# mitrefireline/simfire

Hardware: AMD Instinct MI355X
Metric: cell-updates/sec (grid x envs x steps) (higher is better)
Workload: dtype u8 status + u8 sprite masks + f64 burn_amounts

## Files before the change

profiles/isa_waits.py:

```python
#!/usr/bin/env python3
import argparse
import os
import re
import subprocess
import sys
import tempfile

ROOT = os.path.dirname(os.path.dirname(os.path.abspath(__file__)))
MEM = re.compile(r"^\s*(global_|flat_|scratch_|buffer_|ds_|s_load_|s_buffer_load_)")
LABEL = re.compile(r"^(\.LBB\d+_\d+):")
DPP_START = "wave_shr:1"
ROW_LOAD = "global_load_dwordx4"


def compile_asm(unit, out):
    sys.path.insert(0, ROOT)
    from simfire_amd import build as B
    hipcc = os.environ.get("HIPCC", "/opt/rocm/bin/hipcc")
    flags = [f for f in B.FLAGS if f != "-shared"] + ["-S", "--cuda-device-only"]
    subprocess.run([hipcc] + flags + ["-o", out, os.path.join(B.CSRC, unit)], check=True, stderr=subprocess.DEVNULL)
    return out


def mangled(args):
# ... 65 lines not shown
    skip, every = vm_waits_on_skip_path(body, load, dpp), vm_waits_between(body, load, dpp)
    p("# vmcnt waits between them: %d on the path that takes every s_cbranch_execz, %d on any path" % (len(skip), len(every)))
    p("# index | wait | memory instructions issued since the wait before (x count)")
    pending = []
    for i in range(first, last):
        op = instr(body[i])
        if i == load - 3:
            p("%6d | -- prefetch: the next batch's four rows are requested here" % i)
        if i == dpp:
            p("%6d | -- the batch's work starts (first %s)" % (i, DPP_START))
        if MEM.match(op):
            pending.append(op.split()[0])
        elif op.startswith("s_waitcnt"):
            seen = []
            for m_ in pending:
                if seen and seen[-1][0] == m_:
                    seen[-1][1] += 1
                else:
                    seen.append([m_, 1])
            p("%6d | %-32s | %s" % (i, op, " ".join(n if c == 1 else "%s x%d" % (n, c) for n, c in seen) or "-"))
            pending = []


def main():
    ap = argparse.ArgumentParser(description=__doc__.split("\n")[0])
    ap.add_argument("--unit", default="simfire_hip_run2.hip")
    ap.add_argument("--kernel", default="1,0,1,0,2", help="template arguments of k_run: MAXD,ATT,DIAG,MIT,TEAM")
    ap.add_argument("--asm", default=None)
    a = ap.parse_args()
    if a.asm:
        text = open(a.asm).read()
    else:
        with tempfile.TemporaryDirectory() as d:
            text = open(compile_asm(a.unit, os.path.join(d, "unit.s"))).read()
    report(kernel_lines(text, a.kernel), a.kernel)


if __name__ == "__main__":
    main()
```

simfire_amd/csrc/sf_run_kernels.h:

```cpp
#pragma once

#include "sf_common.h"
#include "sf_step_kernels.h"

namespace {

constexpr int kMarkDw = 32;
constexpr int kStripDw = 19;
#ifdef SF_NO_PERM_ELIG
#define ELIG(x) elig01(x)
#else
#define ELIG(x) elig01_perm(x)
#endif
constexpr int kRunCtl = 24;
constexpr int kRunMaxD = 4;

typedef uint32_t __attribute__((aligned(1))) u32_unaligned;
typedef uint32_t u32x4 __attribute__((ext_vector_type(4)));

__host__ __device__ inline size_t win_lds_bytes(int n_waves)
{
    const int WR = n_waves * 4;
    return (size_t)WR * 64 * 8 + 8 * 8 * 4 + 128 * 4 + 64 * 4 + (size_t)(WR + 2) * 18 * 4 + (size_t)WR * 16 + (size_t)2 * WR * 64 * 2 + (size_t)2 * WR * 64 +
           (size_t)WR * 64 + (size_t)WR * 8 + 256 * 4;
// ... 260 lines not shown
    const void *ka = (const void *)__builtin_amdgcn_kernarg_segment_ptr();
    uint32_t d0 = 0, d1 = 0, d2 = 0, d3 = 0, d4 = 0, d5 = 0, d6 = 0, d7 = 0, d8 = 0, d9 = 0, d10 = 0, d11 = 0, d12 = 0, d13 = 0, d14 = 0, d15 = 0;
    static_assert(BYTES <= 16 * 64, "more lines than this touches");
    d0 = kernarg_line<0>(ka);
    if (BYTES > 1 * 64) d1 = kernarg_line<1 * 64>(ka);
    if (BYTES > 2 * 64) d2 = kernarg_line<2 * 64>(ka);
    if (BYTES > 3 * 64) d3 = kernarg_line<3 * 64>(ka);
    if (BYTES > 4 * 64) d4 = kernarg_line<4 * 64>(ka);
    if (BYTES > 5 * 64) d5 = kernarg_line<5 * 64>(ka);
    if (BYTES > 6 * 64) d6 = kernarg_line<6 * 64>(ka);
    if (BYTES > 7 * 64) d7 = kernarg_line<7 * 64>(ka);
    if (BYTES > 8 * 64) d8 = kernarg_line<8 * 64>(ka);
    if (BYTES > 9 * 64) d9 = kernarg_line<9 * 64>(ka);
    if (BYTES > 10 * 64) d10 = kernarg_line<10 * 64>(ka);
    if (BYTES > 11 * 64) d11 = kernarg_line<11 * 64>(ka);
    if (BYTES > 12 * 64) d12 = kernarg_line<12 * 64>(ka);
    if (BYTES > 13 * 64) d13 = kernarg_line<13 * 64>(ka);
    if (BYTES > 14 * 64) d14 = kernarg_line<14 * 64>(ka);
    if (BYTES > 15 * 64) d15 = kernarg_line<15 * 64>(ka);
    asm volatile("s_waitcnt lgkmcnt(0)" : "+s"(d0), "+s"(d1), "+s"(d2), "+s"(d3), "+s"(d4), "+s"(d5), "+s"(d6), "+s"(d7), "+s"(d8), "+s"(d9), "+s"(d10), "+s"(d11), "+s"(d12),
                 "+s"(d13), "+s"(d14), "+s"(d15));
}

template <int MAXD, int ATT, int DIAG, int MIT, int TEAM = 0>
__global__ __launch_bounds__(1024) void k_run(StepArgs a_by_value, const int n_steps_launch, int vcap, int bsz)
{
    kernarg_touch<(int)sizeof(StepArgs) + 12>();
#ifdef SF_ARGS_BY_VALUE
    constexpr bool kArgsByValue = true;
#else
    constexpr bool kArgsByValue = TEAM == 2 || MIT == -2 || (MIT == 0 && TEAM == 0) || (TEAM == 1 && MAXD == 2);
#endif
    const StepArgs &a = kArgsByValue ? a_by_value : *(const StepArgs *)__builtin_amdgcn_kernarg_segment_ptr();
    extern __shared__ uint4 s_dyn[];
    const Geo &g = a.g;
    const int tid = threadIdx.x, wave = tid >> 6, lane = tid & 63, n_waves = blockDim.x >> 6, nthr = blockDim.x;
    int e_ = 0, tm_ = 0, tn_ = 1;
    bool no_work = false;
    if (TEAM) {
        const uint32_t tt = a.team_tab[blockIdx.x];
        if (tt == kTeamUnused) { if (TEAM != 2) return; no_work = true; }
        else { e_ = (int)(tt & 0xFFFFu); tm_ = (int)((tt >> 16) & 0xFFu); tn_ = (int)(tt >> 24); }
    } else if (a.todo_cnt) {
        const uint32_t n_left = *a.todo_cnt;
        if (blockIdx.x >= n_left) return;
        e_ = (int)a.todo_list[blockIdx.x];
    } else e_ = a.order ? (int)a.order[blockIdx.x] : (int)blockIdx.x;
    int j_s0 = -1;
    for (bool first_pass = true;; first_pass = false) {
    if (TEAM == 2 && (!first_pass || no_work)) {
        if (a.team_recut >= n_steps_launch) return;
        uint32_t *sc = reinterpret_cast<uint32_t *>(s_dyn);
        JoinArgs ja;
        ja.xj = a.xj; ja.xcut = a.xcut; ja.xerr = a.xerr; ja.E = g.E; ja.team_recut = a.team_recut; ja.join_floor = a.join_floor; ja.join_ovh = a.join_ovh;
        ja.team_timeout = a.team_timeout; ja.join_local = a.join_local; ja.t_cap = kTeamMax < g.TY ? kTeamMax : g.TY;
        const uint4 t = find_team(ja, sc);
// ... 169 lines not shown
        }
        __syncthreads();
        R0 = (int)tcnt[0]; R1 = (int)tcnt[1];
        const bool fits = __builtin_amdgcn_readfirstlane((int)tcnt[2]) != 0;
        R0 = __builtin_amdgcn_readfirstlane(R0); R1 = __builtin_amdgcn_readfirstlane(R1);
        if (R1 > g.H) R1 = g.H;
        __syncthreads();
        return fits;
    };
    {
        bool fits = true;
        if (TEAM && (tn > 1 || a.team_rcap) && general) fits = cut_bands(tn > 1 && a.team_recut > 0 && a.team_recut < n_steps ? a.team_recut : n_steps - s_begin);
        if (TEAM && a.todo_out && tm == 0 && tid == 0) a.todo_out[e] = fits ? 0 : n_steps - s_begin;
        if (TEAM && !fits) {
            if (!a.todo_out && tid == 0) *reinterpret_cast<volatile uint32_t *>(a.xerr) = 1u;
            if (s_begin > 0 && tm == 0 && tid == 0) a.commit[e] = st;
            return;
        }
    }
    bool has_up = TEAM && tm > 0, has_dn = TEAM && tm + 1 < tn;
    if (TEAM == 2 && tm == 0 && j_s0 < 0 && tid == 0)
        __hip_atomic_store(a.xj + 2 * g.E + 2 + e, (uint32_t)__builtin_amdgcn_s_getreg((20 << 0) | (0 << 6) | (31 << 11)) & 15u, __ATOMIC_RELAXED, __HIP_MEMORY_SCOPE_AGENT);
    auto team_release = [&]() {
        if (TEAM == 2 && a.join_local == 1) asm volatile("s_waitcnt vmcnt(0)" ::: "memory");
        else __builtin_amdgcn_fence(__ATOMIC_RELEASE, "agent");
    };
    auto team_acquire = [&]() { __builtin_amdgcn_fence(__ATOMIC_ACQUIRE, "agent"); };
    bool one_l2 = false;
    bool gave_up = false;
    auto line_up = [&](const uint32_t tag, const bool report) {
        typedef unsigned long long u64;
        int lane = threadIdx.x & 63;
        asm volatile("" : "+v"(lane));
        const uint32_t xcc = (uint32_t)__builtin_amdgcn_s_getreg((20 << 0) | (0 << 6) | (31 << 11)) & 15u;
        if (lane == 0) __hip_atomic_store(a.xg + ((size_t)e * kTeamMax + tm) * 3 + 2, ((u64)tag << 32) | (u64)xcc, __ATOMIC_RELAXED, __HIP_MEMORY_SCOPE_AGENT);
        u64 x = ((u64)tag << 32) | xcc;
        const unsigned long long t0 = __builtin_amdgcn_s_memrealtime();
        for (;;) {
            if (lane < tn) x = __hip_atomic_load(a.xg + ((size_t)e * kTeamMax + lane) * 3 + 2, __ATOMIC_RELAXED, __HIP_MEMORY_SCOPE_AGENT);
            if (__all((uint32_t)(x >> 32) >= tag)) break;
            __builtin_amdgcn_s_sleep(2);
            if (gave_up || __builtin_amdgcn_s_memrealtime() - t0 > a.team_timeout) {
                if (report) {
                    if (lane == 0) *reinterpret_cast<volatile uint32_t *>(a.xerr) = 1u;
                    gave_up = true;
                }
                break;
            }
        }
        one_l2 = __all((uint32_t)(x >> 32) >= tag && ((uint32_t)x & 15u) == xcc) && !a.team_far;
    };
    unsigned long long *vb = vb0, *vf = nullptr, *vl = nullptr, *ve = nullptr;
    auto load_band = [&]() {
        int tid = threadIdx.x;
        asm volatile("" : "+v"(tid));
        const int yoff = TEAM && a.team_rcap ? R0 - 1 : 0;
        vb = vb0 - (long long)yoff * VW;
        vf = fine ? vb + (size_t)lds_rows * VW : nullptr; vl = fine ? vb + (size_t)2 * lds_rows * VW : nullptr;
        ve = fine ? vb + (size_t)3 * lds_rows * VW : nullptr;
        const int y_lo = TEAM && a.team_rcap ? (R0 > 0 ? R0 - 1 : 0) : 0, y_hi = TEAM && a.team_rcap ? (R1 < g.H ? R1 + 1 : g.H) : g.H;
        for (int i = y_lo * VW + tid; i < y_hi * VW; i += nthr) {
            vb[i] = vb_glob[i];
            if (fine) {
                vf[i] = vb_glob[(long long)g.E * g.vb_env + i];
                vl[i] = vb_glob[2ll * g.E * g.vb_env + i];
                ve[i] = ~0ull;
            }
        }
        if (TEAM && tn > 1) {
            for (int i = tid; i < 2 * g.PV; i += nthr) {
                const int side = i >= g.PV, v = side ? i - g.PV : i, yh = side ? R1 : R0 - 1;
                uint4 r = make_uint4(0, 0, 0, 0);
                if (side ? has_dn : has_up)
                    r = *reinterpret_cast<const uint4 *>(a.cells + (long long)e * g.cells_env + bl_vec(g, yh, v) + (yh & 1) * 16);
                halo[i] = r;
            }
        }
    };
    if (general) load_band();
    PhaseClock pc;
#ifdef SF_PHASES
    uint32_t *ph_acc = ctl + kRunCtl + wave * 16;
    if (lane < 16) ph_acc[lane] = 0;
    pc.start(ph_acc);
#else
    pc.start();
#endif
    __syncthreads();
    if (TEAM == 1 && tn > 1) {
// ... 37 lines not shown
            __syncthreads();
            load_band();
            __syncthreads();
        }
    }
    if (TEAM && tn > 1) {
        if (wave == 0) line_up(TEAM == 2 && j_s0 >= 0 ? 2u + (uint32_t)(j_s0 / a.team_recut) : 1u, TEAM == 2 && j_s0 >= 0);
        if (TEAM == 2) __syncthreads();
    }

    RunEnv ev;
    ev.cells = a.cells + (long long)e * g.cells_env;
    ev.burn = a.burn + (long long)e * g.plane_env;
    ev.settled = a.settled ? a.settled + (long long)e * g.plane_env : nullptr;
    ev.rt = a.rt + (long long)e * g.rt_env;
    ev.vb = vb; ev.vf = vf; ev.vl = vl;
    ev.tdirty = a.tdirty + (long long)e * g.TY * g.TX;
    ev.tot = reinterpret_cast<int32_t *>(ctl + 10);
    int rpt = ((TEAM ? R1 - R0 : g.H) + nthr - 1) / nthr;
    int row0 = TEAM ? R0 : 0;
    auto store_band = [&]() {
        int tid = threadIdx.x;
        asm volatile("" : "+v"(tid));
        for (int i = R0 * VW + tid; i < R1 * VW; i += nthr) {
            vb_glob[i] = vb[i];
            vb_glob[(long long)g.E * g.vb_env + i] = vf[i];
            vb_glob[2ll * g.E * g.vb_env + i] = vl[i];
        }
    };
    const unsigned long long last_word_mask = (g.PV & 63) ? ((1ull << (g.PV & 63)) - 1ull) : ~0ull;

    const bool mit_one_wave = mit && a.mit_k <= 64;
    const int mit_wave = n_waves - 1;
    constexpr bool loop = MIT == -2;
    auto load_pt = [&](int s) {
        if (wave == mit_wave && lane < a.mit_k) {
            const int32_t *p = mit + (((long long)s * g.E + e) * a.mit_k + lane) * 3;
            px = p[0]; py = p[1]; pty = p[2];
        }
    };
    if (mit_one_wave && n_steps > 0 && !loop && !kWinMit) load_pt(0);
    uint32_t lseq = 0;
    if (loop) {
        if (tid == 0) ctl[18] = __hip_atomic_load(a.loop_done + e, __ATOMIC_RELAXED, __HIP_MEMORY_SCOPE_AGENT);
        __syncthreads();
        lseq = (uint32_t)__builtin_amdgcn_readfirstlane((int)ctl[18]);
        n_steps = 0x7FFFFFFF;
        counts_env(g, e, a.status, a.cells, a.tdirty, a.thist, st.running, st.steps, st.elapsed, a.res_block, a.res_elapsed, nullptr,
                   reinterpret_cast<int32_t (*)[6]>(vlist + vcap));
        if (tid == 0)
            for (int q = 0; q < 6; ++q) ev.tot[q] = a.res_block[e * 8 + 2 + q];
        if (e == 0 && a.mit_k > 0 && lseq > 0) {
            const int n16 = g.E * a.mit_k;
            const u32x4 *src = reinterpret_cast<const u32x4 *>(a.loop_pts_host) + (size_t)(lseq & 1u) * n16;
            u32x4 *cpy = reinterpret_cast<u32x4 *>(a.loop_pts) + (size_t)(lseq & 1u) * n16;
            for (int i = tid; i < n16; i += nthr) {
                u32x4 v;
                asm volatile("global_load_dwordx4 %0, %1, off sc0 sc1\n\ts_waitcnt vmcnt(0)" : "=&v"(v) : "v"(src + i) : "memory");
                if (v.w == lseq) asm volatile("global_store_dwordx4 %0, %1, off sc0 sc1" :: "v"(cpy + i), "v"(v) : "memory");
            }
        }
        __syncthreads();
    }
    unsigned long long join_clk = __builtin_readcyclecounter();
    unsigned long long x_clocks = 0;
    uint32_t x_steps = 0;
    for (int s = s_begin; s < n_steps && (st.running || mit); ++s) {
        const int k = s % 3, kn = (s + 1) % 3;
#ifdef SF_PHASES
        pc.tl = (e == g_timeline_env && s == g_timeline_step) ? g_timeline + wave * 64 : nullptr;
#endif
        auto loop_finish = [&]() {
            __syncthreads();
            if (tid == 0) {
                const int32_t *tot = ev.tot;
                int32_t *row = a.res_block + e * 8;
                row[0] = st.running == 1; row[1] = st.steps;
                for (int q = 0; q < 6; ++q) row[2 + q] = tot[q];
                a.res_elapsed[e] = st.elapsed;
            }
            ++lseq;
            if (wave == 0) {
                uint32_t *stage = strips;
                if (lane == 0) {
                    const int32_t *row = a.res_block + e * 8;
                    const unsigned long long el = (unsigned long long)__double_as_longlong(st.elapsed);
                    stage[0] = (uint32_t)row[0]; stage[1] = (uint32_t)row[1]; stage[2] = (uint32_t)row[2];
                    stage[4] = (uint32_t)row[3]; stage[5] = (uint32_t)row[4]; stage[6] = (uint32_t)row[5];
                    stage[8] = (uint32_t)row[6]; stage[9] = (uint32_t)row[7]; stage[10] = (uint32_t)el;
// ... 203 lines not shown
        }
        pc.mark(15);
        if (tid < 3) ctl[3 * tid + kn] = 0;
        const int t = st.steps + 1;
        const Masks mk = make_masks(t, g.md, g.N);
        const bool spread = !st.time_quit;
        const uint32_t L4 = rep4(mk.m_live), EXP4 = rep4(mk.b_exp), CLR4 = rep4(mk.b_clr);
        const int exp_sh = __ffs(mk.b_exp) - 1;
        const uint32_t lo_mask = diag ? L4 : (L4 & 0xFF00FF00u), hi_mask = diag ? L4 : (L4 & 0x00FF00FFu);

        unsigned long long D[MAXD];
        uint32_t cnt = 0;
        if (fine) {
#pragma unroll
            for (int d = 0; d < MAXD; ++d) {
                D[d] = 0;
                const int i = MAXD == 1 ? 0 : d / VW, w = MAXD == 1 ? 0 : d - i * VW;
                const int y = row0 + tid * rpt + i;
                if (i < rpt && y < R1) {
                    int o = y * VW + w;
                    asm volatile("" : "+v"(o));
                    const int up_o = y > 0 ? -VW : 0, dn_o = y + 1 < g.H ? VW : 0;
                    const unsigned long long b1 = vb[o], l1 = vl[o], f1 = vf[o], e1 = ve[o];
                    unsigned long long b02 = 0, l02 = 0, f02 = 0;
                    if (up_o) { b02 = vb[o + up_o]; l02 = vl[o + up_o]; f02 = vf[o + up_o]; }
                    if (dn_o) { b02 |= vb[o + dn_o]; l02 |= vl[o + dn_o]; f02 |= vf[o + dn_o]; }
                    unsigned long long edge = ((l02 | l1) << 1) | ((f02 | f1) >> 1);
                    if (MAXD > 1 && VW > 1) {
                        if (w > 0) edge |= (vl[o - 1] | vl[o - 1 + up_o] | vl[o - 1 + dn_o]) >> 63;
                        if (w + 1 < VW) edge |= (vf[o + 1] | vf[o + 1 + up_o] | vf[o + 1 + dn_o]) << 63;
                    }
                    unsigned long long m = b1 | (e1 & (b02 | edge)) | l02 | f02;
                    if (g.dense) m = ~0ull;
                    if (w == VW - 1) m &= last_word_mask;
                    D[d] = m;
                    cnt += (uint32_t)__popcll(m);
                }
            }
        } else {
#pragma unroll
            for (int d = 0; d < MAXD; ++d) {
                D[d] = 0;
                const int i = d / g.VW, w = d - i * g.VW;
                const int y = tid * rpt + i;
                if (i < rpt && y < g.H) {
                    const unsigned long long *row = vb + y * g.VW;
                    const int up_o = y > 0 ? -g.VW : 0, dn_o = y + 1 < g.H ? g.VW : 0;
                    unsigned long long m = row[w] | row[w + up_o] | row[w + dn_o];
                    m |= (m << 1) | (m >> 1);
                    if (w > 0) m |= (row[w - 1] | row[w - 1 + up_o] | row[w - 1 + dn_o]) >> 63;
                    if (w + 1 < g.VW) m |= (row[w + 1] | row[w + 1 + up_o] | row[w + 1 + dn_o]) << 63;
                    if (g.dense) m = ~0ull;
                    if (w == g.VW - 1) m &= last_word_mask;
                    D[d] = m;
                    cnt += (uint32_t)__popcll(m);
                }
            }
        }
        uint32_t pos0 = 0;
#ifndef SF_NO_SKIP_EMPTY
        if (__ballot(cnt != 0) != 0ull)
#endif
        {
            const uint32_t incl = wave_scan_incl(cnt, lane);
            const uint32_t wave_total = wave_last(incl);
            uint32_t wbase = 0;
            if (lane == 0) wbase = atomicAdd(&ctl[k], wave_total);
            wbase = (uint32_t)__builtin_amdgcn_readfirstlane((int)wbase);
            pos0 = wbase + incl - cnt;
        }
        pc.mark(1);

        uint32_t n_all = 0;
        for (uint32_t cb = 0;; cb += (uint32_t)vcap) {
// ... 238 lines not shown
                    batch(vin_a, ja, vin_b, jb);
                    if (jb >= n_chunk) break;
                    batch(vin_b, jb, vin_a, ja);
                }
            } else {
                for (uint32_t ja = j_first; ja < n_chunk;) {
                    const VecIn cur = vin_a;
                    const uint32_t j0 = ja;
                    batch(cur, j0, vin_a, ja);
                }
            }
            if (cb + (uint32_t)vcap >= n_all) break;
            __syncthreads();
            if (tid == 0) ctl[6 + k] = 0;
        }
        if (TEAM && tn > 1) asm volatile("s_waitcnt vmcnt(0)" ::: "memory");
        __syncthreads();
        pc.mark(0);
        const bool cut_step = TEAM && a.team_recut > 0 && (s + 1) % a.team_recut == 0 && s + 1 < n_steps;
        const bool recut_now = cut_step && tn > 1;
        int tn_new = tn;
        if (TEAM == 2 && cut_step) {
            if (tm == 0 && tid == 0) {
                const uint32_t c = __hip_atomic_load(a.xj + e, __ATOMIC_RELAXED, __HIP_MEMORY_SCOPE_AGENT) & 0xFFu;
                const uint32_t t_cap = (uint32_t)(kTeamMax < g.TY ? kTeamMax : g.TY);
                ctl[20] = c > t_cap ? t_cap : (c < (uint32_t)tn ? (uint32_t)tn : c);
                const unsigned long long now = __builtin_readcyclecounter();
                long long per = (long long)((now - join_clk) / (unsigned long long)a.team_recut);
                join_clk = now;
                if (tn > 1) per = (per - a.join_ovh) * tn;
                if (per < a.join_floor) per = a.join_floor;
                const long long left = n_steps - (s + 1);
                const uint32_t b = (uint32_t)((per >> 4) > 0x3FFFF ? 0x3FFFF : (per >> 4)) << 14 | (uint32_t)(left > 0x3FFF ? 0x3FFF : left);
                __hip_atomic_store(a.xj + g.E + e, b, __ATOMIC_RELAXED, __HIP_MEMORY_SCOPE_AGENT);
            }
            if (!recut_now) __syncthreads();
        }
        if (recut_now) {
            store_band();
            team_release();
            __syncthreads();
        }
        if (TEAM == 2 && cut_step && tm == 0) tn_new = __builtin_amdgcn_readfirstlane((int)ctl[20]);
        if (TEAM && tn > 1) {
            if (wave == 0) {
                typedef unsigned long long u64;
                int lane = threadIdx.x & 63;
// ... 24 lines not shown
                asm volatile("s_waitcnt vmcnt(0)" ::: "memory");
                if (lane == 0) {
                    const u64 gv = ((u64)epoch << 32) | (u64)(ctl[3 + k] & 0xFFFFu) | (TEAM == 2 ? (u64)tn_new << 16 : 0ull);
                    if (one_l2) __hip_atomic_store(a.xg + ((size_t)e * kTeamMax + tm) * 3 + par, gv, __ATOMIC_RELAXED, __HIP_MEMORY_SCOPE_WORKGROUP);
                    else __hip_atomic_store(a.xg + ((size_t)e * kTeamMax + tm) * 3 + par, gv, __ATOMIC_RELAXED, __HIP_MEMORY_SCOPE_AGENT);
                }
                u64 x = (u64)epoch << 32;
                {
                    const unsigned long long t0 = __builtin_amdgcn_s_memrealtime();
                    for (;;) {
                        if (lane < tn) x = __hip_atomic_load(a.xg + ((size_t)e * kTeamMax + lane) * 3 + par, __ATOMIC_RELAXED, __HIP_MEMORY_SCOPE_AGENT);
                        if (__all((uint32_t)(x >> 32) == epoch)) break;
                        __builtin_amdgcn_s_sleep(1);
                        if (gave_up || __builtin_amdgcn_s_memrealtime() - t0 > a.team_timeout) {
                            if (lane == 0) *reinterpret_cast<volatile uint32_t *>(a.xerr) = 1u;
                            gave_up = true;
                            break;
                        }
                    }
                }
                const bool live_any = __ballot(lane < tn && (x & 0xFFull)) != 0ull, cand_any = __ballot(lane < tn && (x & 0xFF00ull)) != 0ull;
                if (lane == 0) ctl[3 + k] = (live_any ? FLAG_LIVE : 0u) | (cand_any ? FLAG_CAND : 0u);
                if (TEAM == 2 && cut_step && lane == 0) ctl[20] = (uint32_t)(x >> 16) & 0xFFu;
                for (int side = 0; side < 2 && one_l2; ++side) {
                    if (!(side ? has_dn : has_up)) continue;
                    const int yh = side ? R1 : R0 - 1;
                    for (int v0 = 0; v0 < g.PV; v0 += 64) {
                        const int v = v0 + lane;
                        u64 lo = 0, hi = 0;
                        if (v < g.PV) {
                            const u64 *src = reinterpret_cast<const u64 *>(ev.cells + bl_vec(g, yh, v) + (yh & 1) * 16);
                            lo = __hip_atomic_load(src, __ATOMIC_RELAXED, __HIP_MEMORY_SCOPE_AGENT);
                            hi = __hip_atomic_load(src + 1, __ATOMIC_RELAXED, __HIP_MEMORY_SCOPE_AGENT);
                        }
                        if (v < g.PV) halo[side * g.PV + v] = make_uint4((uint32_t)lo, (uint32_t)(lo >> 32), (uint32_t)hi, (uint32_t)(hi >> 32));
                        const u64 bw = __ballot((lo | hi) != 0ull), fw = __ballot((lo & 0xFFull) != 0ull), lw = __ballot((hi >> 56) != 0ull);
                        if (lane == 0) { vb[yh * VW + (v0 >> 6)] = bw; vf[yh * VW + (v0 >> 6)] = fw; vl[yh * VW + (v0 >> 6)] = lw; }
                    }
                }
                for (int side = 0; side < 2 && !one_l2; ++side) {
                    if (!(side ? has_dn : has_up)) continue;
                    const int nj = side ? tm + 1 : tm - 1, yh = side ? R1 : R0 - 1;
                    const u64 *src = reinterpret_cast<const u64 *>(a.xbuf + ((size_t)(e * kTeamMax + nj) * 4 + (size_t)((side ^ 1) * 2 + par)) * a.xrow);
                    u64 word = 0;
                    if (lane < 3 * VW) word = __hip_atomic_load(src + lane, __ATOMIC_RELAXED, __HIP_MEMORY_SCOPE_AGENT);
                    for (int v0 = 0; v0 < g.PV; v0 += 64) {
                        const int v = v0 + lane;
                        u64 lo = 0, hi = 0;
                        if (v < g.PV) {
                            lo = __hip_atomic_load(src + 8 + v * 2, __ATOMIC_RELAXED, __HIP_MEMORY_SCOPE_AGENT);
                            hi = __hip_atomic_load(src + 8 + v * 2 + 1, __ATOMIC_RELAXED, __HIP_MEMORY_SCOPE_AGENT);
                        }
                        const int wl = v0 >> 6;
                        const u64 bw = (u64)(uint32_t)__builtin_amdgcn_readlane((int)(uint32_t)word, wl) |
                                       ((u64)(uint32_t)__builtin_amdgcn_readlane((int)(uint32_t)(word >> 32), wl) << 32);
                        if (v < g.PV) {
                            const bool on = (bw >> lane) & 1ull;
                            halo[side * g.PV + v] = on ? make_uint4((uint32_t)lo, (uint32_t)(lo >> 32), (uint32_t)hi, (uint32_t)(hi >> 32)) : make_uint4(0, 0, 0, 0);
                        }
                    }
                    if (lane < 3 * VW) {
                        const int which = lane / VW, w = lane - which * VW;
                        (which == 0 ? vb : (which == 1 ? vf : vl))[yh * VW + w] = word;
                    }
                }
                if (a.counters && lane == 0) { x_clocks += __builtin_readcyclecounter() - xt0; x_steps++; }
            }
            __builtin_amdgcn_fence(__ATOMIC_RELEASE, "workgroup", "local");
            __builtin_amdgcn_s_barrier();
            __builtin_amdgcn_fence(__ATOMIC_ACQUIRE, "workgroup", "local");
        }
        st = fold_state(st, ctl[3 + k], g);
        st.running = __builtin_amdgcn_readfirstlane(st.running);
        st.steps = __builtin_amdgcn_readfirstlane(st.steps);
        st.complete = __builtin_amdgcn_readfirstlane(st.complete);
        st.time_quit = __builtin_amdgcn_readfirstlane(st.time_quit);
        if (loop) loop_finish();
        if (TEAM == 2 && cut_step && tn > 1) tn_new = __builtin_amdgcn_readfirstlane((int)ctl[20]);
        if (TEAM == 2 && gave_up) tn_new = tn;
        if ((recut_now || tn_new > tn) && (st.running || mit)) {
            if (TEAM == 2 && tn == 1) {
                store_band();
                team_release();
                __syncthreads();
            }
            if (TEAM == 2 && tn_new > tn && tm == 0 && tid == 0) {
                a.commit[e] = st;
                team_release();
                __hip_atomic_store(a.xcut + e, ((unsigned long long)tn_new << 24) | (unsigned long long)(s + 1), __ATOMIC_RELAXED, __HIP_MEMORY_SCOPE_AGENT);
                atomicAdd(a.xj + 2 * g.E + 1, (uint32_t)(tn_new - tn));
                const uint32_t li = atomicAdd(a.jlog, 1u);
                if (li < (uint32_t)kJoinLog) { a.jlog[1 + 3 * li] = (uint32_t)e; a.jlog[2 + 3 * li] = (uint32_t)(s + 1); a.jlog[3 + 3 * li] = (uint32_t)tn_new; }
            }
            team_acquire();
            if (TEAM == 2) { tn = tn_new; has_up = tm > 0; has_dn = tm + 1 < tn; }
            const int left = n_steps - (s + 1);
            cut_bands(a.team_recut < left ? a.team_recut : left);
            load_band();
            ev.vb = vb; ev.vf = vf; ev.vl = vl;
            rpt = (R1 - R0 + nthr - 1) / nthr;
            row0 = R0;
            __syncthreads();
            if (wave == 0) line_up(2u + (uint32_t)((s + 1) / a.team_recut), true);
// ... 30 lines not shown
            else a.cost[e] = c32;
        }
    }
    if (TEAM) {
        if (general) store_band();
    } else if (general) {
        for (int i = tid; i < n_words; i += nthr) vb_glob[i] = vb[i];
        if (fine)
            for (int i = tid; i < g.H; i += nthr) {
                vb_glob[(long long)g.E * g.vb_env + i] = vf[i];
                vb_glob[2ll * g.E * g.vb_env + i] = vl[i];
            }
    }
    wpc.note(49);
    if (a.counters && lane == 0) {
        int cw = wave;
        asm volatile("" : "+v"(cw));
        unsigned long long *cs = a.counters + (size_t)((blockIdx.x * 16 + cw) & (kCounterShards - 1)) * kCounterRow;
        if (n_active) atomicAdd(&cs[0], (unsigned long long)n_active);
        if (n_ignite) atomicAdd(&cs[1], (unsigned long long)n_ignite);
        if (n_items_acc) atomicAdd(&cs[2], (unsigned long long)n_items_acc);
        if (n_phase2) atomicAdd(&cs[4], (unsigned long long)n_phase2);
        if (n_vec_done) atomicAdd(&cs[5], (unsigned long long)n_vec_done);
        if (TEAM && x_steps) {
            atomicAdd(&cs[6], (unsigned long long)x_steps | ((unsigned long long)(one_l2 ? x_steps : 0u) << 32));
            atomicAdd(&cs[7], x_clocks);
        }
    }
    if (TEAM && tn > 1) {
        __syncthreads();
        if (tid == 0) {
            __builtin_amdgcn_fence(__ATOMIC_RELEASE, "agent");
            asm volatile("s_waitcnt vmcnt(0)" ::: "memory");
            const uint32_t before = atomicAdd(&a.xdone[e], 1u);
            const bool last = before == (uint32_t)tn - 1u;
            if (last) __builtin_amdgcn_fence(__ATOMIC_ACQUIRE, "agent");
            ctl[0] = last ? 1u : 0u;
        }
        __syncthreads();
        if (!ctl[0]) {
            if (TEAM == 2) continue;
            return;
        }
    }
    if (a.res_block && !(win_result && !general) && !(a.row_valid && !general && n_steps == 0 && !mit)) {
        __syncthreads();
        wpc.note(36);
        counts_env(g, e, a.status, a.cells, a.tdirty, a.thist, st.running, st.steps, st.elapsed, a.res_block, a.res_elapsed, a.res_sink,
                   reinterpret_cast<int32_t (*)[6]>(vlist + vcap));
// ... 218 lines not shown
```

Baseline: 23980 billion.

## Cut register pressure and batch loads in team step-boundary and band paths

Cold kernel arguments used in the team paths (load_band, store_band, recut, team_release) are now re-read through the kernarg pointer, behind an opaque zero offset, instead of being held live across the step loop. The per-wave exchange counters move from registers into LDS ctl slots. The band load loop handles two elements per iteration, and the halo exchange issues the up and down row loads together before consuming them. Neighbour-word LDS reads in the edge computation are grouped with asm barriers. The aim is fewer spills (readlane/writelane) in the step loop and more memory-level parallelism at step boundaries, at the cost of extra kernarg scalar loads and LDS atomics on the counter path. A profiling script adds a report on this part of the step loop.

```diff
diff --git a/profiles/isa_waits.py b/profiles/isa_waits.py
--- a/profiles/isa_waits.py
+++ b/profiles/isa_waits.py
@@ -111,18 +111,239 @@
             pending = []
 
 
+BB_COMMENT = re.compile(r"^; %bb\.\d+:")
+SPILL_OPS = ("v_readlane_b32", "v_writelane_b32", "s_nop")
+
+
+def kernel_blocks(asm_text, args):
+    key = mangled(args)
+    lines = asm_text.splitlines()
+    start = next((i for i, ln in enumerate(lines) if key in ln and re.match(r"^_Z\S+:", ln)), None)
+    if start is None:
+        raise LookupError("no k_run<%s> in this assembly" % args)
+    end = next(i for i in range(start, len(lines)) if lines[i].startswith(".Lfunc_end"))
+    body, blocks, parent, notes = [], [], {}, None
+
+    def close():
+        if notes is None:
+            return
+        first, name, text = notes
+        ups = re.findall(r"Parent Loop (BB\d+_\d+) Depth=", text)
+        member = re.search(r"in Loop: Header=(BB\d+_\d+) ", text)
+        if "Loop Header: Depth=" in text and name:
+            parent[name] = ups[-1] if ups else None
+            blocks.append((first, name))
+        else:
+            blocks.append((first, member.group(1) if member else None))
+
+    for ln in lines[start + 1:end]:
+        if not ln.strip():
+            continue
+        m = LABEL.match(ln)
+        if m or BB_COMMENT.match(ln):
+            close()
+            notes = [len(body), m.group(1)[2:] if m else None, ln]
+            if m:
+                body.append(ln)
+        elif ln.lstrip().startswith(";"):
+            if notes is not None and notes[0] == len(body) - (1 if notes[1] else 0):
+                notes[2] += "\n" + ln
+        else:
+            body.append(ln)
+    close()
+    return body, blocks, parent
+
+
+def _inside(loop, hdr, parent):
+    while loop is not None:
+        if loop == hdr:
+            return True
+        loop = parent.get(loop)
+    return False
+
+
+def step_chain(body, blocks, parent):
+    batch = loop_range(body, find_prefetch(body)[1])[2]
+    step = parent[parent[batch]]
+    if step is None:
+        raise LookupError("the batch loop %s has no loop two levels out" % batch)
+    spans = []
+    for n, (first, loop) in enumerate(blocks):
+        last = blocks[n + 1][0] if n + 1 < len(blocks) else len(body)
+        if _inside(loop, step, parent) and not _inside(loop, batch, parent) and last > first:
+            if spans and spans[-1][1] == first:
+                spans[-1][1] = last
+            else:
+                spans.append([first, last])
+    return step, batch, [tuple(sp) for sp in spans]
+
+
+def step_own_blocks(body, step):
+    labs = [i for i, ln in enumerate(body) if LABEL.match(ln)] + [len(body)]
+    return [i for a, b in zip(labs, labs[1:]) if ("Header=%s " % step) in body[a] for i in range(a, b)]
+
+
+def chain_indices(spans):
+    return [i for first, last in spans for i in range(first, last)]
+
+
+def count_ops(body, idx):
+    out = dict.fromkeys(SPILL_OPS, 0)
+    out["all"] = 0
+    for i in idx:
+        if LABEL.match(body[i]):
+            continue
+        out["all"] += 1
+        op = instr(body[i]).split()[0]
+        if op in out:
+            out[op] += 1
+    return out
+
+
+def waits(body, idx):
+    out, pending = [], []
+    for i in idx:
+        if LABEL.match(body[i]):
+            continue
+        op = instr(body[i])
+        if MEM.match("\t" + op):
+            pending.append(op)
+        elif op.startswith("s_waitcnt") or op.startswith("s_barrier"):
+            out.append((i, op, pending))
+            pending = []
+    return out
+
+
+def interest_pass(body, spans):
+    idx = chain_indices(spans)
+    stop = next(n for n, i in enumerate(idx) if instr(body[i]).startswith("ds_add_rtn_u32"))
+    return idx[:stop]
+
+
+def is_sc1_row_load(op):
+    return op.startswith("global_load_dwordx2") and " sc1" in op and " sc0" not in op
+
+
+def boundary_paths(body, spans):
+    idx = chain_indices(spans)
+    loads = [i for i in idx if is_sc1_row_load(instr(body[i]))]
+    off = lambda i: int((re.search(r"offset:(\d+)", instr(body[i])) or [0, 0])[1])
+    base = lambda i: instr(body[i]).split(",")[1].strip()
+    paths = {"one_l2": [], "written_through": []}
+    for a, b in zip(loads, loads[1:]):
+        if base(a) == base(b) and off(b) == off(a) + 8 and b - a <= 4:
+            paths["written_through" if off(a) >= 64 else "one_l2"] += [a, b]
+    return paths
+
+
+def loads_before_first_wait(body, idx, start, is_load, counter="vmcnt"):
+    n = 0
+    for i in idx[idx.index(start):]:
+        op = instr(body[i])
+        if op.startswith("s_waitcnt") and counter in op:
+            break
+        if not LABEL.match(body[i]) and is_load(op):
+            n += 1
+    return n
+
+
+def is_plain_word_load(op):
+    return op.startswith("global_load_dwordx2") and " sc" not in op and " nt" not in op
+
+
+def band_load_loop(body, blocks, parent, spans):
+    step, batch, _ = step_chain(body, blocks, parent)
+    per_loop = {}
+    for n, (first, loop) in enumerate(blocks):
+        last = blocks[n + 1][0] if n + 1 < len(blocks) else len(body)
+        if loop not in (None, step) and _inside(loop, step, parent) and not _inside(loop, batch, parent):
+            per_loop.setdefault(loop, []).extend(range(first, last))
+    for loop, idx in per_loop.items():
+        ops = [instr(body[i]) for i in idx if not LABEL.match(body[i])]
+        if any(is_plain_word_load(o) for o in ops) and any(o.startswith("ds_write_b64") or o.startswith("ds_write2_b64") for o in ops) and \
+                not any(o.startswith("global_store") or o.startswith("global_atomic") for o in ops):
+            return idx
+    raise LookupError("no loop with plain 8-byte loads and 8-byte LDS stores in the step chain")
+
+
+def _short(ops):
+    seen = []
+    for o in ops:
+        n = o.split()[0] + (" sc1" if " sc1" in o else "")
+        if seen and seen[-1][0] == n:
+            seen[-1][1] += 1
+        else:
+            seen.append([n, 1])
+    return " ".join(n if c == 1 else "%s x%d" % (n, c) for n, c in seen) or "-"
+
+
+def report_chain(asm_text, args, out=sys.stdout):
+    body, blocks, parent = kernel_blocks(asm_text, args)
+    step, batch, spans = step_chain(body, blocks, parent)
+    idx = chain_indices(spans)
+    p = lambda *a: print(*a, file=out)
+    c = count_ops(body, idx)
+    p("# k_run<%s>: step loop = loop with header %s, batch loop = %s; the step loop outside the batch loop:" % (args.replace(",", ", "), step, batch))
+    p("#   %d instructions in %d runs of blocks; v_readlane_b32 %d, v_writelane_b32 %d, s_nop %d" %
+      (c["all"], len(spans), c["v_readlane_b32"], c["v_writelane_b32"], c["s_nop"]))
+    cb = count_ops(body, range(*loop_range(body, find_prefetch(body)[1])[:2]))
+    co = count_ops(body, step_own_blocks(body, step))
+    p("#   of these in the labelled blocks of the step loop's own depth (no inner loop): %d instructions; v_readlane_b32 %d, v_writelane_b32 %d, s_nop %d" %
+      (co["all"], co["v_readlane_b32"], co["v_writelane_b32"], co["s_nop"]))
+    p("#   (the batch loop itself: %d instructions, v_readlane_b32 %d, v_writelane_b32 %d, s_nop %d)" % (cb["all"], cb["v_readlane_b32"], cb["v_writelane_b32"], cb["s_nop"]))
+    marks = {}
+    ip = interest_pass(body, spans)
+    marks[ip[0]] = "step start: interest pass"
+    marks[ip[-1] + 1] = "interest pass ends (the wave's range of the vector list)"
+    ws = waits(body, ip)
+    p("#   interest pass %d .. %d: %d waits that name lgkmcnt with exactly one ds_read since the wait before" %
+      (ip[0], ip[-1], sum(1 for _, op, pend in ws if "lgkmcnt" in op and sum(o.startswith("ds_read") for o in pend) == 1)))
+    try:
+        for name, loads in boundary_paths(body, spans).items():
+            if loads:
+                marks[loads[0]] = "step boundary, %s path: first row load" % name
+                p("#   step boundary, %s path: %d sc1 row loads, %d of them in front of the first vmcnt wait" %
+                  (name, len(loads), loads_before_first_wait(body, idx, loads[0], is_sc1_row_load)))
+        bl = band_load_loop(body, blocks, parent, spans)
+        marks[bl[0]] = "load_band: loop over the bitmap words"
+        p("#   load_band's loop %d .. %d: %d plane loads in front of the first vmcnt wait" % (bl[0], bl[-1], loads_before_first_wait(body, bl, bl[0], is_plain_word_load)))
+    except (LookupError, StopIteration) as ex:
+        p("#   (no team code found: %s)" % ex)
+    p("# index | wait or barrier | memory instructions issued since the one before (x count)")
+    pending, prev_last = [], None
+    for first, last in spans:
+        if prev_last is not None:
+            p("       | -- blocks %d .. %d are not part of the chain (batch loop or outside the step loop)" % (prev_last, first - 1))
+        prev_last = last
+        for i in range(first, last):
+            if i in marks:
+                p("%6d | -- %s" % (i, marks[i]))
+            if LABEL.match(body[i]):
+                continue
+            op = instr(body[i])
+            if MEM.match("\t" + op):
+                pending.append(op)
+            elif op.startswith("s_waitcnt") or op.startswith("s_barrier"):
+                p("%6d | %-32s | %s" % (i, op, _short(pending)))
+                pending = []
+
+
 def main():
     ap = argparse.ArgumentParser(description=__doc__.split("\n")[0])
     ap.add_argument("--unit", default="simfire_hip_run2.hip")
     ap.add_argument("--kernel", default="1,0,1,0,2", help="template arguments of k_run: MAXD,ATT,DIAG,MIT,TEAM")
     ap.add_argument("--asm", default=None)
+    ap.add_argument("--chain", action="store_true", help="the second report: the step loop outside the batch loop")
     a = ap.parse_args()
     if a.asm:
         text = open(a.asm).read()
     else:
         with tempfile.TemporaryDirectory() as d:
             text = open(compile_asm(a.unit, os.path.join(d, "unit.s"))).read()
-    report(kernel_lines(text, a.kernel), a.kernel)
+    if a.chain:
+        report_chain(text, a.kernel)
+    else:
+        report(kernel_lines(text, a.kernel), a.kernel)
 
 
 if __name__ == "__main__":
diff --git a/simfire_amd/csrc/sf_run_kernels.h b/simfire_amd/csrc/sf_run_kernels.h
--- a/simfire_amd/csrc/sf_run_kernels.h
+++ b/simfire_amd/csrc/sf_run_kernels.h
@@ -306,6 +306,15 @@
                  "+s"(d13), "+s"(d14), "+s"(d15));
 }
 
+template <int TEAM>
+__device__ __forceinline__ const StepArgs &cold_args(const StepArgs &a)
+{
+    if (TEAM == 0) return a;
+    long z = 0;
+    asm volatile("" : "+s"(z));
+    return *(const StepArgs *)((const char *)__builtin_amdgcn_kernarg_segment_ptr() + z);
+}
+
 template <int MAXD, int ATT, int DIAG, int MIT, int TEAM = 0>
 __global__ __launch_bounds__(1024) void k_run(StepArgs a_by_value, const int n_steps_launch, int vcap, int bsz)
 {
@@ -316,6 +325,7 @@
     constexpr bool kArgsByValue = TEAM == 2 || MIT == -2 || (MIT == 0 && TEAM == 0) || (TEAM == 1 && MAXD == 2);
 #endif
     const StepArgs &a = kArgsByValue ? a_by_value : *(const StepArgs *)__builtin_amdgcn_kernarg_segment_ptr();
+    const StepArgs &a_hot = a;
     extern __shared__ uint4 s_dyn[];
     const Geo &g = a.g;
     const int tid = threadIdx.x, wave = tid >> 6, lane = tid & 63, n_waves = blockDim.x >> 6, nthr = blockDim.x;
@@ -531,7 +541,7 @@
     if (TEAM == 2 && tm == 0 && j_s0 < 0 && tid == 0)
         __hip_atomic_store(a.xj + 2 * g.E + 2 + e, (uint32_t)__builtin_amdgcn_s_getreg((20 << 0) | (0 << 6) | (31 << 11)) & 15u, __ATOMIC_RELAXED, __HIP_MEMORY_SCOPE_AGENT);
     auto team_release = [&]() {
-        if (TEAM == 2 && a.join_local == 1) asm volatile("s_waitcnt vmcnt(0)" ::: "memory");
+        if (TEAM == 2 && cold_args<TEAM>(a_hot).join_local == 1) asm volatile("s_waitcnt vmcnt(0)" ::: "memory");
         else __builtin_amdgcn_fence(__ATOMIC_RELEASE, "agent");
     };
     auto team_acquire = [&]() { __builtin_amdgcn_fence(__ATOMIC_ACQUIRE, "agent"); };
@@ -541,6 +551,7 @@
         typedef unsigned long long u64;
         int lane = threadIdx.x & 63;
         asm volatile("" : "+v"(lane));
+        const StepArgs &a = cold_args<TEAM>(a_hot);
         const uint32_t xcc = (uint32_t)__builtin_amdgcn_s_getreg((20 << 0) | (0 << 6) | (31 << 11)) & 15u;
         if (lane == 0) __hip_atomic_store(a.xg + ((size_t)e * kTeamMax + tm) * 3 + 2, ((u64)tag << 32) | (u64)xcc, __ATOMIC_RELAXED, __HIP_MEMORY_SCOPE_AGENT);
         u64 x = ((u64)tag << 32) | xcc;
@@ -563,17 +574,29 @@
     auto load_band = [&]() {
         int tid = threadIdx.x;
         asm volatile("" : "+v"(tid));
+        const StepArgs &a = cold_args<TEAM>(a_hot);
+        const Geo &g = a.g;
+        const unsigned long long *vb_glob = a.vbits + (long long)e * g.vb_env;
         const int yoff = TEAM && a.team_rcap ? R0 - 1 : 0;
         vb = vb0 - (long long)yoff * VW;
         vf = fine ? vb + (size_t)lds_rows * VW : nullptr; vl = fine ? vb + (size_t)2 * lds_rows * VW : nullptr;
         ve = fine ? vb + (size_t)3 * lds_rows * VW : nullptr;
         const int y_lo = TEAM && a.team_rcap ? (R0 > 0 ? R0 - 1 : 0) : 0, y_hi = TEAM && a.team_rcap ? (R1 < g.H ? R1 + 1 : g.H) : g.H;
-        for (int i = y_lo * VW + tid; i < y_hi * VW; i += nthr) {
-            vb[i] = vb_glob[i];
-            if (fine) {
-                vf[i] = vb_glob[(long long)g.E * g.vb_env + i];
-                vl[i] = vb_glob[2ll * g.E * g.vb_env + i];
-                ve[i] = ~0ull;
+        for (int i = y_lo * VW + tid; i < y_hi * VW; i += 2 * nthr) {
+            const int i2 = i + nthr;
+            const bool two = i2 < y_hi * VW;
+            unsigned long long b_a = vb_glob[i], f_a = 0, l_a = 0, b_b = 0, f_b = 0, l_b = 0;
+            if (fine) { f_a = vb_glob[(long long)g.E * g.vb_env + i]; l_a = vb_glob[2ll * g.E * g.vb_env + i]; }
+            if (two) {
+                b_b = vb_glob[i2];
+                if (fine) { f_b = vb_glob[(long long)g.E * g.vb_env + i2]; l_b = vb_glob[2ll * g.E * g.vb_env + i2]; }
+            }
+            asm volatile("" : "+v"(b_a), "+v"(f_a), "+v"(l_a), "+v"(b_b), "+v"(f_b), "+v"(l_b));
+            vb[i] = b_a;
+            if (fine) { vf[i] = f_a; vl[i] = l_a; ve[i] = ~0ull; }
+            if (two) {
+                vb[i2] = b_b;
+                if (fine) { vf[i2] = f_b; vl[i2] = l_b; ve[i2] = ~0ull; }
             }
         }
         if (TEAM && tn > 1) {
@@ -657,10 +680,15 @@
     auto store_band = [&]() {
         int tid = threadIdx.x;
         asm volatile("" : "+v"(tid));
+        const StepArgs &a = cold_args<TEAM>(a_hot);
+        const Geo &g = a.g;
+        unsigned long long *vb_glob = a.vbits + (long long)e * g.vb_env;
         for (int i = R0 * VW + tid; i < R1 * VW; i += nthr) {
-            vb_glob[i] = vb[i];
-            vb_glob[(long long)g.E * g.vb_env + i] = vf[i];
-            vb_glob[2ll * g.E * g.vb_env + i] = vl[i];
+            unsigned long long b = vb[i], f = vf[i], l = vl[i];
+            asm volatile("" : "+v"(b), "+v"(f), "+v"(l));
+            vb_glob[i] = b;
+            vb_glob[(long long)g.E * g.vb_env + i] = f;
+            vb_glob[2ll * g.E * g.vb_env + i] = l;
         }
     };
     const unsigned long long last_word_mask = (g.PV & 63) ? ((1ull << (g.PV & 63)) - 1ull) : ~0ull;
@@ -698,8 +726,7 @@
         __syncthreads();
     }
     unsigned long long join_clk = __builtin_readcyclecounter();
-    unsigned long long x_clocks = 0;
-    uint32_t x_steps = 0;
+    if (TEAM && tid == 0) { ctl[9] = 0; ctl[22] = 0; ctl[23] = 0; }
     for (int s = s_begin; s < n_steps && (st.running || mit); ++s) {
         const int k = s % 3, kn = (s + 1) % 3;
 #ifdef SF_PHASES
@@ -949,13 +976,18 @@
                     asm volatile("" : "+v"(o));
                     const int up_o = y > 0 ? -VW : 0, dn_o = y + 1 < g.H ? VW : 0;
                     const unsigned long long b1 = vb[o], l1 = vl[o], f1 = vf[o], e1 = ve[o];
-                    unsigned long long b02 = 0, l02 = 0, f02 = 0;
-                    if (up_o) { b02 = vb[o + up_o]; l02 = vl[o + up_o]; f02 = vf[o + up_o]; }
-                    if (dn_o) { b02 |= vb[o + dn_o]; l02 |= vl[o + dn_o]; f02 |= vf[o + dn_o]; }
+                    unsigned long long b0 = 0, l0 = 0, f0 = 0, b2 = 0, l2 = 0, f2 = 0;
+                    if (up_o) { b0 = vb[o + up_o]; l0 = vl[o + up_o]; f0 = vf[o + up_o]; }
+                    if (dn_o) { b2 = vb[o + dn_o]; l2 = vl[o + dn_o]; f2 = vf[o + dn_o]; }
+                    asm volatile("" : "+v"(b0), "+v"(l0), "+v"(f0), "+v"(b2), "+v"(l2), "+v"(f2));
+                    const unsigned long long b02 = b0 | b2, l02 = l0 | l2, f02 = f0 | f2;
                     unsigned long long edge = ((l02 | l1) << 1) | ((f02 | f1) >> 1);
                     if (MAXD > 1 && VW > 1) {
-                        if (w > 0) edge |= (vl[o - 1] | vl[o - 1 + up_o] | vl[o - 1 + dn_o]) >> 63;
-                        if (w + 1 < VW) edge |= (vf[o + 1] | vf[o + 1 + up_o] | vf[o + 1 + dn_o]) << 63;
+                        unsigned long long pl0 = 0, pl1 = 0, pl2 = 0, nf0 = 0, nf1 = 0, nf2 = 0;
+                        if (w > 0) { pl1 = vl[o - 1]; pl0 = vl[o - 1 + up_o]; pl2 = vl[o - 1 + dn_o]; }
+                        if (w + 1 < VW) { nf1 = vf[o + 1]; nf0 = vf[o + 1 + up_o]; nf2 = vf[o + 1 + dn_o]; }
+                        asm volatile("" : "+v"(pl0), "+v"(pl1), "+v"(pl2), "+v"(nf0), "+v"(nf1), "+v"(nf2));
+                        edge |= ((pl1 | pl0 | pl2) >> 63) | ((nf1 | nf0 | nf2) << 63);
                     }
                     unsigned long long m = b1 | (e1 & (b02 | edge)) | l02 | f02;
                     if (g.dense) m = ~0ull;
@@ -973,10 +1005,14 @@
                 if (i < rpt && y < g.H) {
                     const unsigned long long *row = vb + y * g.VW;
                     const int up_o = y > 0 ? -g.VW : 0, dn_o = y + 1 < g.H ? g.VW : 0;
-                    unsigned long long m = row[w] | row[w + up_o] | row[w + dn_o];
+                    unsigned long long c1 = row[w], c0 = row[w + up_o], c2 = row[w + dn_o];
+                    unsigned long long p0 = 0, p1 = 0, p2 = 0, n0 = 0, n1 = 0, n2 = 0;
+                    if (w > 0) { p1 = row[w - 1]; p0 = row[w - 1 + up_o]; p2 = row[w - 1 + dn_o]; }
+                    if (w + 1 < g.VW) { n1 = row[w + 1]; n0 = row[w + 1 + up_o]; n2 = row[w + 1 + dn_o]; }
+                    asm volatile("" : "+v"(c0), "+v"(c1), "+v"(c2), "+v"(p0), "+v"(p1), "+v"(p2), "+v"(n0), "+v"(n1), "+v"(n2));
+                    unsigned long long m = c1 | c0 | c2;
                     m |= (m << 1) | (m >> 1);
-                    if (w > 0) m |= (row[w - 1] | row[w - 1 + up_o] | row[w - 1 + dn_o]) >> 63;
-                    if (w + 1 < g.VW) m |= (row[w + 1] | row[w + 1 + up_o] | row[w + 1 + dn_o]) << 63;
+                    m |= ((p1 | p0 | p2) >> 63) | ((n1 | n0 | n2) << 63);
                     if (g.dense) m = ~0ull;
                     if (w == g.VW - 1) m &= last_word_mask;
                     D[d] = m;
@@ -1261,7 +1297,9 @@
         int tn_new = tn;
         if (TEAM == 2 && cut_step) {
             if (tm == 0 && tid == 0) {
-                const uint32_t c = __hip_atomic_load(a.xj + e, __ATOMIC_RELAXED, __HIP_MEMORY_SCOPE_AGENT) & 0xFFu;
+                const StepArgs &a = cold_args<TEAM>(a_hot);
+                const Geo &g = a.g;
+                const uint32_t c = __hip_atomic_load(a.xj + e, __ATOMIC_RELAXED, __HIP_MEMORY_SCOPE_AGENT) & 0xFFFFu;
                 const uint32_t t_cap = (uint32_t)(kTeamMax < g.TY ? kTeamMax : g.TY);
                 ctl[20] = c > t_cap ? t_cap : (c < (uint32_t)tn ? (uint32_t)tn : c);
                 const unsigned long long now = __builtin_readcyclecounter();
@@ -1332,49 +1370,79 @@
                 const bool live_any = __ballot(lane < tn && (x & 0xFFull)) != 0ull, cand_any = __ballot(lane < tn && (x & 0xFF00ull)) != 0ull;
                 if (lane == 0) ctl[3 + k] = (live_any ? FLAG_LIVE : 0u) | (cand_any ? FLAG_CAND : 0u);
                 if (TEAM == 2 && cut_step && lane == 0) ctl[20] = (uint32_t)(x >> 16) & 0xFFu;
-                for (int side = 0; side < 2 && one_l2; ++side) {
-                    if (!(side ? has_dn : has_up)) continue;
-                    const int yh = side ? R1 : R0 - 1;
+                if (one_l2) {
                     for (int v0 = 0; v0 < g.PV; v0 += 64) {
                         const int v = v0 + lane;
-                        u64 lo = 0, hi = 0;
+                        u64 lo_u = 0, hi_u = 0, lo_d = 0, hi_d = 0;
                         if (v < g.PV) {
-                            const u64 *src = reinterpret_cast<const u64 *>(ev.cells + bl_vec(g, yh, v) + (yh & 1) * 16);
-                            lo = __hip_atomic_load(src, __ATOMIC_RELAXED, __HIP_MEMORY_SCOPE_AGENT);
-                            hi = __hip_atomic_load(src + 1, __ATOMIC_RELAXED, __HIP_MEMORY_SCOPE_AGENT);
+                            const uint32_t vo = (uint32_t)v * 128u;
+                            if (has_up) {
+                                const u64 *src = reinterpret_cast<const u64 *>(ev.cells + bl_vec(g, R0 - 1, 0) + ((R0 - 1) & 1) * 16 + vo);
+                                lo_u = __hip_atomic_load(src, __ATOMIC_RELAXED, __HIP_MEMORY_SCOPE_AGENT);
+                                hi_u = __hip_atomic_load(src + 1, __ATOMIC_RELAXED, __HIP_MEMORY_SCOPE_AGENT);
+                            }
+                            if (has_dn) {
+                                const u64 *src = reinterpret_cast<const u64 *>(ev.cells + bl_vec(g, R1, 0) + (R1 & 1) * 16 + vo);
+                                lo_d = __hip_atomic_load(src, __ATOMIC_RELAXED, __HIP_MEMORY_SCOPE_AGENT);
+                                hi_d = __hip_atomic_load(src + 1, __ATOMIC_RELAXED, __HIP_MEMORY_SCOPE_AGENT);
+                            }
                         }
-                        if (v < g.PV) halo[side * g.PV + v] = make_uint4((uint32_t)lo, (uint32_t)(lo >> 32), (uint32_t)hi, (uint32_t)(hi >> 32));
-                        const u64 bw = __ballot((lo | hi) != 0ull), fw = __ballot((lo & 0xFFull) != 0ull), lw = __ballot((hi >> 56) != 0ull);
-                        if (lane == 0) { vb[yh * VW + (v0 >> 6)] = bw; vf[yh * VW + (v0 >> 6)] = fw; vl[yh * VW + (v0 >> 6)] = lw; }
-                    }
-                }
-                for (int side = 0; side < 2 && !one_l2; ++side) {
-                    if (!(side ? has_dn : has_up)) continue;
-                    const int nj = side ? tm + 1 : tm - 1, yh = side ? R1 : R0 - 1;
-                    const u64 *src = reinterpret_cast<const u64 *>(a.xbuf + ((size_t)(e * kTeamMax + nj) * 4 + (size_t)((side ^ 1) * 2 + par)) * a.xrow);
-                    u64 word = 0;
-                    if (lane < 3 * VW) word = __hip_atomic_load(src + lane, __ATOMIC_RELAXED, __HIP_MEMORY_SCOPE_AGENT);
+                        int lane_c = threadIdx.x & 63;
+                        asm volatile("" : "+v"(lo_u), "+v"(hi_u), "+v"(lo_d), "+v"(hi_d), "+v"(lane_c));
+                        for (int side = 0; side < 2; ++side) {
+                            if (!(side ? has_dn : has_up)) continue;
+                            const int yh = side ? R1 : R0 - 1, v = v0 + lane_c, lane = lane_c;
+                            const u64 lo = side ? lo_d : lo_u, hi = side ? hi_d : hi_u;
+                            if (v < g.PV) halo[side * g.PV + v] = make_uint4((uint32_t)lo, (uint32_t)(lo >> 32), (uint32_t)hi, (uint32_t)(hi >> 32));
+                            const u64 bw = __ballot((lo | hi) != 0ull), fw = __ballot((lo & 0xFFull) != 0ull), lw = __ballot((hi >> 56) != 0ull);
+                            if (lane == 0) { vb[yh * VW + (v0 >> 6)] = bw; vf[yh * VW + (v0 >> 6)] = fw; vl[yh * VW + (v0 >> 6)] = lw; }
+                        }
+                    }
+                } else {
+                    const u64 *src_u = reinterpret_cast<const u64 *>(a.xbuf + ((size_t)(e * kTeamMax + (has_up ? tm - 1 : tm)) * 4 + (size_t)(1 * 2 + par)) * a.xrow);
+                    const u64 *src_d = reinterpret_cast<const u64 *>(a.xbuf + ((size_t)(e * kTeamMax + (has_dn ? tm + 1 : tm)) * 4 + (size_t)(0 * 2 + par)) * a.xrow);
+                    u64 word_u = 0, word_d = 0;
+                    if (has_up && lane < 3 * VW) word_u = __hip_atomic_load(src_u + lane, __ATOMIC_RELAXED, __HIP_MEMORY_SCOPE_AGENT);
+                    if (has_dn && lane < 3 * VW) word_d = __hip_atomic_load(src_d + lane, __ATOMIC_RELAXED, __HIP_MEMORY_SCOPE_AGENT);
                     for (int v0 = 0; v0 < g.PV; v0 += 64) {
                         const int v = v0 + lane;
-                        u64 lo = 0, hi = 0;
+                        u64 lo_u = 0, hi_u = 0, lo_d = 0, hi_d = 0;
                         if (v < g.PV) {
-                            lo = __hip_atomic_load(src + 8 + v * 2, __ATOMIC_RELAXED, __HIP_MEMORY_SCOPE_AGENT);
-                            hi = __hip_atomic_load(src + 8 + v * 2 + 1, __ATOMIC_RELAXED, __HIP_MEMORY_SCOPE_AGENT);
+                            const uint32_t vo = (uint32_t)v * 2u;
+                            if (has_up) {
+                                lo_u = __hip_atomic_load(src_u + 8 + vo, __ATOMIC_RELAXED, __HIP_MEMORY_SCOPE_AGENT);
+                                hi_u = __hip_atomic_load(src_u + 8 + vo + 1, __ATOMIC_RELAXED, __HIP_MEMORY_SCOPE_AGENT);
+                            }
+                            if (has_dn) {
+                                lo_d = __hip_atomic_load(src_d + 8 + vo, __ATOMIC_RELAXED, __HIP_MEMORY_SCOPE_AGENT);
+                                hi_d = __hip_atomic_load(src_d + 8 + vo + 1, __ATOMIC_RELAXED, __HIP_MEMORY_SCOPE_AGENT);
+                            }
                         }
+                        int lane_c = threadIdx.x & 63;
+                        asm volatile("" : "+v"(word_u), "+v"(word_d), "+v"(lo_u), "+v"(hi_u), "+v"(lo_d), "+v"(hi_d), "+v"(lane_c));
                         const int wl = v0 >> 6;
-                        const u64 bw = (u64)(uint32_t)__builtin_amdgcn_readlane((int)(uint32_t)word, wl) |
-                                       ((u64)(uint32_t)__builtin_amdgcn_readlane((int)(uint32_t)(word >> 32), wl) << 32);
-                        if (v < g.PV) {
-                            const bool on = (bw >> lane) & 1ull;
-                            halo[side * g.PV + v] = on ? make_uint4((uint32_t)lo, (uint32_t)(lo >> 32), (uint32_t)hi, (uint32_t)(hi >> 32)) : make_uint4(0, 0, 0, 0);
+                        for (int side = 0; side < 2; ++side) {
+                            if (!(side ? has_dn : has_up)) continue;
+                            const int v = v0 + lane_c, lane = lane_c;
+                            const u64 word = side ? word_d : word_u, lo = side ? lo_d : lo_u, hi = side ? hi_d : hi_u;
+                            const u64 bw = (u64)(uint32_t)__builtin_amdgcn_readlane((int)(uint32_t)word, wl) |
+                                           ((u64)(uint32_t)__builtin_amdgcn_readlane((int)(uint32_t)(word >> 32), wl) << 32);
+                            if (v < g.PV) {
+                                const bool on = (bw >> lane) & 1ull;
+                                halo[side * g.PV + v] = on ? make_uint4((uint32_t)lo, (uint32_t)(lo >> 32), (uint32_t)hi, (uint32_t)(hi >> 32)) : make_uint4(0, 0, 0, 0);
+                            }
                         }
                     }
                     if (lane < 3 * VW) {
                         const int which = lane / VW, w = lane - which * VW;
-                        (which == 0 ? vb : (which == 1 ? vf : vl))[yh * VW + w] = word;
-                    }
-                }
-                if (a.counters && lane == 0) { x_clocks += __builtin_readcyclecounter() - xt0; x_steps++; }
+                        if (has_up) (which == 0 ? vb : (which == 1 ? vf : vl))[(R0 - 1) * VW + w] = word_u;
+                        if (has_dn) (which == 0 ? vb : (which == 1 ? vf : vl))[R1 * VW + w] = word_d;
+                    }
+                }
+                if (a.counters && lane == 0) {
+                    atomicAdd(reinterpret_cast<unsigned long long *>(ctl + 22), (unsigned long long)(__builtin_readcyclecounter() - xt0));
+                    atomicAdd(ctl + 9, 1u);
+                }
             }
             __builtin_amdgcn_fence(__ATOMIC_RELEASE, "workgroup", "local");
             __builtin_amdgcn_s_barrier();
@@ -1389,6 +1457,8 @@
         if (TEAM == 2 && cut_step && tn > 1) tn_new = __builtin_amdgcn_readfirstlane((int)ctl[20]);
         if (TEAM == 2 && gave_up) tn_new = tn;
         if ((recut_now || tn_new > tn) && (st.running || mit)) {
+            const StepArgs &a = cold_args<TEAM>(a_hot);
+            const Geo &g = a.g;
             if (TEAM == 2 && tn == 1) {
                 store_band();
                 team_release();
@@ -1465,9 +1535,10 @@
         if (n_items_acc) atomicAdd(&cs[2], (unsigned long long)n_items_acc);
         if (n_phase2) atomicAdd(&cs[4], (unsigned long long)n_phase2);
         if (n_vec_done) atomicAdd(&cs[5], (unsigned long long)n_vec_done);
+        const uint32_t x_steps = TEAM && cw == 0 ? ctl[9] : 0u;
         if (TEAM && x_steps) {
             atomicAdd(&cs[6], (unsigned long long)x_steps | ((unsigned long long)(one_l2 ? x_steps : 0u) << 32));
-            atomicAdd(&cs[7], x_clocks);
+            atomicAdd(&cs[7], *reinterpret_cast<unsigned long long *>(ctl + 22));
         }
     }
     if (TEAM && tn > 1) {
```

Result: slower. 23700 billion (-1.1%).
